# LabJunBMI/E3-invaraint-diffusion-model

Hardware: NVIDIA B200
Metric: denoiser graph-steps/s (forward + reverse-diffusion step per pocket graph; cfg2: 64 pockets x 500 steps, L=128) (higher is better)
Workload: dtype bf16

## Files before the change

### e3-invaraint-diffusion-model_b200/csrc/gemm.cu

```cuda
#include <cstdio>
#include <cstdlib>
#include <mutex>
#include <type_traits>
#include <unordered_map>

#include "common.cuh"
#include "kernels.h"

namespace seqdiff {

typedef CUresult (*PFN_encodeTiled)(CUtensorMap*, CUtensorMapDataType, cuuint32_t, void*, const cuuint64_t*,
                                    const cuuint64_t*, const cuuint32_t*, const cuuint32_t*, CUtensorMapInterleave,
                                    CUtensorMapSwizzle, CUtensorMapL2promotion, CUtensorMapFloatOOBfill);

static PFN_encodeTiled get_encode_fn() {
  static PFN_encodeTiled fn = nullptr;
  static std::once_flag once;
  std::call_once(once, [] {
    void* p = nullptr;
    cudaDriverEntryPointQueryResult qres;
    if (cudaGetDriverEntryPoint("cuTensorMapEncodeTiled", &p, cudaEnableDefault, &qres) == cudaSuccess &&
        qres == cudaDriverEntryPointSuccess)
      fn = reinterpret_cast<PFN_encodeTiled>(p);
  });
// ... 55 lines not shown
  static std::mutex mu;
  static std::unordered_map<TmapKey, CUtensorMap, TmapKeyHash> cache;
  TmapKey key{ptr, rows, cols, -32, fmt};
  {
    std::lock_guard<std::mutex> g(mu);
    auto it = cache.find(key);
    if (it != cache.end()) {
      *out = it->second;
      return SEQDIFF_OK;
    }
  }
  PFN_encodeTiled enc = get_encode_fn();
  if (!enc) {
    set_error("cuTensorMapEncodeTiled not available from the driver");
    return SEQDIFF_ERR_CUDA;
  }
  SD_CHECK((reinterpret_cast<uintptr_t>(ptr) & 15) == 0 && (cols % 32) == 0, "TMA store operand must be 16B aligned with N a multiple of 32");
  cuuint64_t gdim[2] = {static_cast<cuuint64_t>(cols), static_cast<cuuint64_t>(rows)};
  cuuint64_t gstride[1] = {static_cast<cuuint64_t>(cols) * 2};
  cuuint32_t box[2] = {32u, 32u};
  cuuint32_t estr[2] = {1u, 1u};
  CUresult r = enc(out, fmt == 1 ? CU_TENSOR_MAP_DATA_TYPE_BFLOAT16 : CU_TENSOR_MAP_DATA_TYPE_FLOAT16, 2, const_cast<void*>(ptr), gdim,
                   gstride, box, estr, CU_TENSOR_MAP_INTERLEAVE_NONE, CU_TENSOR_MAP_SWIZZLE_64B, CU_TENSOR_MAP_L2_PROMOTION_NONE,
                   CU_TENSOR_MAP_FLOAT_OOB_FILL_NONE);
  if (r != CUDA_SUCCESS) {
    set_error("cuTensorMapEncodeTiled (store) failed with CUresult " + std::to_string(static_cast<int>(r)));
    return SEQDIFF_ERR_CUDA;
  }
  std::lock_guard<std::mutex> g(mu);
  cache.emplace(key, *out);
  return SEQDIFF_OK;
}

int make_tmap_3d(const void* ptr, int fmt, int batch, int rows, int cols, int box_rows, CUtensorMap* out) {
  PFN_encodeTiled enc = get_encode_fn();
  if (!enc) {
    set_error("cuTensorMapEncodeTiled not available from the driver");
    return SEQDIFF_ERR_CUDA;
  }
  SD_CHECK((reinterpret_cast<uintptr_t>(ptr) & 15) == 0 && (cols % 8) == 0, "TMA operand must be 16B aligned with a 16B-multiple row pitch");
  cuuint64_t gdim[3] = {static_cast<cuuint64_t>(cols), static_cast<cuuint64_t>(rows), static_cast<cuuint64_t>(batch)};
  cuuint64_t gstride[2] = {static_cast<cuuint64_t>(cols) * 2, static_cast<cuuint64_t>(rows) * cols * 2};
  cuuint32_t box[3] = {64u, static_cast<cuuint32_t>(box_rows), 1u};
  cuuint32_t estr[3] = {1u, 1u, 1u};
  CUresult r = enc(out, fmt == 1 ? CU_TENSOR_MAP_DATA_TYPE_BFLOAT16 : CU_TENSOR_MAP_DATA_TYPE_FLOAT16, 3, const_cast<void*>(ptr), gdim,
                   gstride, box, estr, CU_TENSOR_MAP_INTERLEAVE_NONE, CU_TENSOR_MAP_SWIZZLE_128B, CU_TENSOR_MAP_L2_PROMOTION_L2_256B,
                   CU_TENSOR_MAP_FLOAT_OOB_FILL_NONE);
  if (r != CUDA_SUCCESS) {
    set_error("cuTensorMapEncodeTiled (3d) failed with CUresult " + std::to_string(static_cast<int>(r)));
    return SEQDIFF_ERR_CUDA;
  }
  return SEQDIFF_OK;
}

constexpr int kBM = 128;
constexpr int kBK = 64;
constexpr int kUmmaK = 16;
constexpr int kGemmThreads = 320;

template <int BN, bool CG2, bool LN = false> struct GemmCfg {
  static constexpr int kNSub = BN > 256 ? 2 : 1;
  static constexpr int kSubN = BN / kNSub;
  static constexpr int kBoxRows = CG2 ? kSubN / 2 : kSubN;
  static constexpr int kBRows = kBoxRows * kNSub;
  static constexpr int kAccStages = BN > 256 ? 1 : 2;
  static constexpr int kABytes = kBM * kBK * 2;
  static constexpr int kBBytes = kBRows * kBK * 2;
  static constexpr int kStageBytes = kABytes + kBBytes;
  static constexpr int kStages = BN > 256 ? 4 : (CG2 ? 6 : (BN == 256 ? (LN ? 3 : 4) : (BN == 192 ? 4 : (LN ? 5 : 6))));
  static constexpr int kTmemCols = BN == 128 ? 256 : 512;
  static constexpr int kStagingBytes = 8 * 32 * 32 * 4;
  static constexpr int kLnBytes = 2 * 128 * 8 + 2 * 4 * 128 * 8 + 64;
  static constexpr int kSmemBytes = kStages * kStageBytes + 1024  + 256  + kStagingBytes + (LN ? kLnBytes : 0);
  static_assert(BN <= 256 || CG2, "tiles wider than one UMMA are built for CTA pairs only");
  static_assert(kSmemBytes <= 232448, "over the 227 KB shared-memory limit");
};

template <typename T> __device__ __forceinline__ void store4(T* p, const float4& v);
template <> __device__ __forceinline__ void store4<float>(float* p, const float4& v) { *reinterpret_cast<float4*>(p) = v; }
template <> __device__ __forceinline__ void store4<bf16>(bf16* p, const float4& v) {
  *reinterpret_cast<uint2*>(p) = make_uint2(pack_bf16x2(v.x, v.y), pack_bf16x2(v.z, v.w));
}
template <> __device__ __forceinline__ void store4<f16>(f16* p, const float4& v) {
  *reinterpret_cast<uint2*>(p) = make_uint2(pack_f16x2(v.x, v.y), pack_f16x2(v.z, v.w));
}

template <typename T> __device__ __forceinline__ void add4(T*, const float4&) {}
template <> __device__ __forceinline__ void add4<float>(float* p, const float4& v) { atomicAdd(reinterpret_cast<float4*>(p), v); }

constexpr int kLnCl = 4;
struct LnOutArgs {
  const float* g;
  const float* b;
  float eps;
  void* h;
  float2* stats;
};
template <int BN, int EPI, int RESID, typename TOut, bool CG2, typename TH = void, bool TN = false>
__global__ void __launch_bounds__(kGemmThreads, 1)
gemm_tcgen05_kernel(const __grid_constant__ CUtensorMap tmA, const __grid_constant__ CUtensorMap tmB, const __grid_constant__ CUtensorMap tmC,
                    const float* __restrict__ bias, const float* __restrict__ resid, TOut* __restrict__ C, int M, int N, int K,
                    uint32_t idesc, const float2* __restrict__ ln_stats, const float* __restrict__ ln_g, const float* __restrict__ ln_b,
                    unsigned long long* __restrict__ trace, const LnOutArgs lno, int l2_stream, int ksplit) {
  constexpr bool LNOUT = !std::is_void<TH>::value;
  using Cfg = GemmCfg<BN, CG2, LNOUT>;
  static_assert(!LNOUT || (!CG2 && RESID != 0 && EPI == 0 && std::is_same<TOut, float>::value), "fused LayerNorm: 1-CTA MMA, fp32 C with residual");
  static_assert(!TN || (!CG2 && !LNOUT && RESID == 0 && EPI == 0 && std::is_same<TOut, float>::value && BN % 64 == 0 && BN <= 256), "TN: 1-CTA MMA, fp32 C");
  constexpr int STAGES = Cfg::kStages;
  constexpr int TILE_M = CG2 ? 2 * kBM : kBM;
  extern __shared__ uint8_t smem_raw[];
  uint8_t* smem = smem_raw + ((1024u - (smem_u32(smem_raw) & 1023u)) & 1023u);
  uint8_t* sA = smem;
  uint8_t* sB = smem + STAGES * Cfg::kABytes;
  uint64_t* bars = reinterpret_cast<uint64_t*>(smem + STAGES * Cfg::kStageBytes);
  uint64_t* full_bar = bars;
  uint64_t* empty_bar = bars + STAGES;
  uint64_t* tfull_bar = bars + 2 * STAGES;
  uint64_t* tempty_bar = bars + 2 * STAGES + 2;
  uint32_t* tmem_slot = reinterpret_cast<uint32_t*>(bars + 2 * STAGES + 4);

  const int warp = warp_id_uniform();
  const int lane = threadIdx.x & 31;
  const int num_n = N / BN;
  const int num_m = (M + TILE_M - 1) / TILE_M;
  const int num_tiles = num_m * num_n * ksplit;
  const int num_kb = (K + kBK - 1) / kBK;
  auto kb_lo = [&](int ks) { return static_cast<int>(static_cast<long long>(num_kb) * ks / ksplit); };
  const uint32_t cta_rank = CG2 ? cluster_ctarank() : 0u;
  const int tile0 = CG2 ? static_cast<int>(blockIdx.x >> 1) : static_cast<int>(blockIdx.x);
  const int tile_step = CG2 ? static_cast<int>(gridDim.x >> 1) : static_cast<int>(gridDim.x);
  float2* ln_cpart = reinterpret_cast<float2*>(smem + STAGES * Cfg::kStageBytes + 256 + Cfg::kStagingBytes);
  float2* ln_xpart = ln_cpart + 2 * 128;
  uint64_t* ln_bar = reinterpret_cast<uint64_t*>(ln_xpart + 2 * 4 * 128);

  int tr_n = 0;
  const bool tr_on = trace != nullptr && blockIdx.x == 0 && lane == 0 && (warp == 0 || warp == 1 || warp == 2 || warp == 6);
  const int tr_base = (warp == 0 ? 0 : warp == 1 ? 1 : warp == 2 ? 2 : 3) * 1024;
  auto TR = [&](int id) {
    if (tr_on && tr_n < 1023) trace[tr_base + 1 + tr_n++] = (static_cast<unsigned long long>(clock64()) << 8) | static_cast<unsigned>(id);
  };
  TR(40);
  if (warp == 0 && lane == 0) {
    tma_prefetch_desc(&tmA);
    tma_prefetch_desc(&tmB);
    if (!std::is_same<TOut, float>::value) tma_prefetch_desc(&tmC);
    for (int i = 0; i < STAGES; ++i) {
      mbar_init(&full_bar[i], 1);
      mbar_init(&empty_bar[i], 1);
    }
    for (int i = 0; i < 2; ++i) {
      mbar_init(&tfull_bar[i], 1);
      mbar_init(&tempty_bar[i], CG2 ? 16 : 8);
      if (LNOUT) mbar_init(&ln_bar[i], kLnCl * 128);
    }
    fence_mbar_init();
  }
  if (warp == 1) {
    if (CG2) {
      tmem_alloc_cg2(tmem_slot, Cfg::kTmemCols);
      tmem_relinquish_cg2();
    } else {
      tmem_alloc(tmem_slot, Cfg::kTmemCols);
      tmem_relinquish();
    }
  }
  tc_fence_before();
  if (CG2 || LNOUT) cluster_sync_all(); else __syncthreads();
  tc_fence_after();
  const uint32_t tmem_base = *tmem_slot;
  TR(41);
  pdl_trigger();
  pdl_wait();
  TR(42);

  if (warp == 0) {
    {
      const uint64_t pol_keep = l2_stream ? l2_policy_evict_last() : 0ull;
      int stage = 0;
      uint32_t phase = 0;
      for (int tile = tile0; tile < num_tiles; tile += tile_step) {
        const int ks = tile % ksplit, mn = tile / ksplit;
        const int m_blk = mn / num_n, n_blk = mn % num_n;
        const int a_row = m_blk * TILE_M + static_cast<int>(cta_rank) * kBM;
        for (int kb = kb_lo(ks), kb_end = kb_lo(ks + 1); kb < kb_end; ++kb) {
          mbar_wait(&empty_bar[stage], phase ^ 1);
          TR(1);
          if (CG2) {
// ... 38 lines not shown
      uint32_t phase = 0;
      int as = 0;
      uint32_t aphase = 0;
      for (int tile = tile0; tile < num_tiles; tile += tile_step) {
        mbar_wait(&tempty_bar[as], aphase ^ 1);
        tc_fence_after();
        const uint32_t tmem_d = tmem_base + static_cast<uint32_t>(as * BN);
        const int kb_begin = kb_lo(tile % ksplit), kb_end = kb_lo(tile % ksplit + 1);
        for (int kb = kb_begin; kb < kb_end; ++kb) {
          mbar_wait(&full_bar[stage], phase);
          tc_fence_after();
          TR(11);
          const uint32_t a_addr = smem_u32(sA + stage * Cfg::kABytes);
          const uint32_t b_addr = smem_u32(sB + stage * Cfg::kBBytes);
#pragma unroll
          for (int k = 0; k < kBK / kUmmaK; ++k) {
            const uint64_t adesc = TN ? umma_desc_mnmajor_sw128(a_addr + k * 2048, 8192) : umma_desc_kmajor_sw128(a_addr + k * kUmmaK * 2);
#pragma unroll
            for (int j = 0; j < Cfg::kNSub; ++j) {
              const uint64_t bdesc = TN ? umma_desc_mnmajor_sw128(b_addr + k * 2048, 8192)
                                        : umma_desc_kmajor_sw128(b_addr + j * Cfg::kBoxRows * kBK * 2 + k * kUmmaK * 2);
              if (CG2) umma_cg2_e(tmem_d + j * Cfg::kSubN, adesc, bdesc, idesc, ((kb - kb_begin) | k) != 0 ? 1u : 0u);
              else umma_bf16_e(tmem_d + j * Cfg::kSubN, adesc, bdesc, idesc, ((kb - kb_begin) | k) != 0 ? 1u : 0u);
            }
          }
          if (CG2) umma_commit_mc_e(&empty_bar[stage], 3); else umma_commit_e(&empty_bar[stage]);
          if (++stage == STAGES) { stage = 0; phase ^= 1; }
        }
        if (CG2) umma_commit_mc_e(&tfull_bar[as], 3); else umma_commit_e(&tfull_bar[as]);
        TR(12);
        if (++as == Cfg::kAccStages) { as = 0; aphase ^= 1; }
      }
    }
  } else {
    const int q = warp & 3;
    const int half = (warp - 2) >> 2;
    float* stage = reinterpret_cast<float*>(smem + STAGES * Cfg::kStageBytes + 256) + (warp - 2) * 1024;
    const int lr = lane >> 3, lc = lane & 7;
    int as = 0;
    uint32_t aphase = 0;
    int ln_it = 0;
    (void)ln_it;
    constexpr bool kTmaOut = !std::is_same<TOut, float>::value && RESID == 0;
    int pcount = 0;
    (void)pcount;
    const uint64_t pol_stream = (kTmaOut && l2_stream) ? l2_policy_evict_first() : 0ull;
    (void)pol_stream;
    constexpr int NCH = BN / 64;
    for (int tile = tile0; tile < num_tiles; tile += tile_step) {
      const int ks = tile % ksplit, mn = tile / ksplit;
      const int m_blk = mn / num_n, n_blk = mn % num_n;
      const int row_base = m_blk * TILE_M + static_cast<int>(cta_rank) * kBM + q * 32;
      SD_DEV_ASSERT(m_blk < num_m && n_blk * BN + half * (BN / 2) + (BN / 2) <= N && ks < ksplit);
      const uint32_t t_row = tmem_base + (static_cast<uint32_t>(q * 32) << 16) + static_cast<uint32_t>(as * BN) + half * (BN / 2);
      const int col0 = n_blk * BN + half * (BN / 2) + 4 * lc;
      const bool full = row_base + 32 <= M;
      float rs[LNOUT ? 8 : 1], rq[LNOUT ? 8 : 1];
      if (LNOUT) {
#pragma unroll
        for (int i = 0; i < 8; ++i) { rs[i] = 0.f; rq[i] = 0.f; }
      }
      (void)rs; (void)rq;
      if constexpr (kTmaOut) {
        const int colw = n_blk * BN + half * (BN / 2);
        uint8_t* panels = reinterpret_cast<uint8_t*>(stage);
        TR(20);
        mbar_wait(&tfull_bar[as], aphase);
        tc_fence_after();
        TR(21);
        uint32_t r[2][32];
        tmem_ld_32x32(t_row, r[0]);
#pragma unroll
        for (int ci = 0; ci < NCH; ++ci) {
          const int cur = ci & 1;
          float4 bv[8];
#pragma unroll
          for (int j4 = 0; j4 < 8; ++j4) bv[j4] = __ldg(reinterpret_cast<const float4*>(bias + colw + 32 * ci + 4 * j4));
          tmem_ld_wait();
          if (ci + 1 < NCH) tmem_ld_32x32(t_row + static_cast<uint32_t>(32 * (ci + 1)), r[cur ^ 1]);
          uint32_t pk[16];
#pragma unroll
          for (int j4 = 0; j4 < 8; ++j4) {
            float a0 = __uint_as_float(r[cur][4 * j4]) + bv[j4].x, a1 = __uint_as_float(r[cur][4 * j4 + 1]) + bv[j4].y;
            float a2 = __uint_as_float(r[cur][4 * j4 + 2]) + bv[j4].z, a3 = __uint_as_float(r[cur][4 * j4 + 3]) + bv[j4].w;
            if (EPI == 1) { a0 = gelu_fast(a0); a1 = gelu_fast(a1); a2 = gelu_fast(a2); a3 = gelu_fast(a3); }
            if (EPI == 2) { a0 = silu_fast(a0); a1 = silu_fast(a1); a2 = silu_fast(a2); a3 = silu_fast(a3); }
            pk[2 * j4] = pack2<TOut>(a0, a1);
            pk[2 * j4 + 1] = pack2<TOut>(a2, a3);
          }
          uint8_t* panel = panels + (pcount & 1) * 2048;
          if (lane == 0) tma_store_wait_read1();
          __syncwarp();
          uint8_t* prow = panel + lane * 64;
          const uint32_t sw = (smem_u32(prow) >> 7) & 3u;
#pragma unroll
// ... 54 lines not shown
#pragma unroll
        for (int jj = 0; jj < 8; ++jj)
          *reinterpret_cast<uint4*>(stage + lane * 32 + ((jj ^ (lane & 7)) << 2)) =
              make_uint4(r[tc][4 * jj], r[tc][4 * jj + 1], r[tc][4 * jj + 2], r[tc][4 * jj + 3]);
        __syncwarp();
        const int col = col0 + 32 * ci;
        auto emit_rows = [&](auto guard_tag) {
          constexpr bool kGuard = decltype(guard_tag)::value;
#pragma unroll
          for (int hh = 0; hh < 2; ++hh) {
            float4 v[4];
#pragma unroll
            for (int u = 0; u < 4; ++u) {
              const int rr = 4 * (4 * hh + u) + lr;
              v[u] = *reinterpret_cast<const float4*>(stage + rr * 32 + ((lc ^ (rr & 7)) << 2));
            }
#pragma unroll
            for (int u = 0; u < 4; ++u) {
              const int i = 4 * hh + u;
              v[u].x += b4[cur].x; v[u].y += b4[cur].y; v[u].z += b4[cur].z; v[u].w += b4[cur].w;
              if (EPI == 1) { v[u].x = gelu_fast(v[u].x); v[u].y = gelu_fast(v[u].y); v[u].z = gelu_fast(v[u].z); v[u].w = gelu_fast(v[u].w); }
              if (EPI == 2) { v[u].x = silu_fast(v[u].x); v[u].y = silu_fast(v[u].y); v[u].z = silu_fast(v[u].z); v[u].w = silu_fast(v[u].w); }
              if (RESID) {
                float4 rv = rres[i];
                if (ci + 1 < NCH) fetch_resid_row(ci + 1, i);
                if (RESID == 2) {
                  rv.x = (rv.x - st8[i].x) * st8[i].y * g4[cur].x + h4[cur].x;
                  rv.y = (rv.y - st8[i].x) * st8[i].y * g4[cur].y + h4[cur].y;
                  rv.z = (rv.z - st8[i].x) * st8[i].y * g4[cur].z + h4[cur].z;
                  rv.w = (rv.w - st8[i].x) * st8[i].y * g4[cur].w + h4[cur].w;
                }
                v[u].x += rv.x; v[u].y += rv.y; v[u].z += rv.z; v[u].w += rv.w;
              }
              if (LNOUT) {
                rs[i] += (v[u].x + v[u].y) + (v[u].z + v[u].w);
                rq[i] = fmaf(v[u].x, v[u].x, fmaf(v[u].y, v[u].y, fmaf(v[u].z, v[u].z, fmaf(v[u].w, v[u].w, rq[i]))));
              }
            }
#pragma unroll
            for (int u = 0; u < 4; ++u) {
              const int row = row_base + 4 * (4 * hh + u) + lr;
              if (!kGuard || row < M) {
                if (std::is_same<TOut, float>::value && RESID == 0 && ksplit > 1) add4(C + static_cast<size_t>(row) * N + col, v[u]);
                else store4<TOut>(C + static_cast<size_t>(row) * N + col, v[u]);
              }
            }
          }
        };
        if (full) emit_rows(std::false_type{}); else emit_rows(std::true_type{});
        __syncwarp();
      }
      }
      TR(23);
      tc_fence_before();
      __syncwarp();
      if (lane == 0) {
        if (CG2 && cta_rank != 0) mbar_arrive_cluster(mapa_u32(smem_u32(&tempty_bar[as]), 0));
        else mbar_arrive(&tempty_bar[as]);
      }
      if constexpr (LNOUT) {
        const int et = static_cast<int>(threadIdx.x) - 64;
        const int par = ln_it & 1;
        float4 vc[NCH][8];
#pragma unroll
        for (int ci = 0; ci < NCH; ++ci)
#pragma unroll
          for (int i = 0; i < 8; ++i) {
            const int row = row_base + 4 * i + lr;
            vc[ci][i] = (full || row < M) ? *reinterpret_cast<const float4*>(C + static_cast<size_t>(row) * N + col0 + 32 * ci)
                                          : make_float4(0.f, 0.f, 0.f, 0.f);
          }
#pragma unroll
        for (int i = 0; i < 8; ++i)
#pragma unroll
          for (int off = 1; off < 8; off <<= 1) {
            rs[i] += __shfl_xor_sync(0xffffffffu, rs[i], off);
            rq[i] += __shfl_xor_sync(0xffffffffu, rq[i], off);
          }
        if (lc == 0) {
#pragma unroll
          for (int i = 0; i < 8; ++i) ln_cpart[half * 128 + q * 32 + 4 * i + lr] = make_float2(rs[i], rq[i]);
        }
        asm volatile("bar.sync 1, 256;" ::: "memory");
        if (et < 128) {
          const float2 a = ln_cpart[et], b2 = ln_cpart[128 + et];
          const uint32_t my = cluster_ctarank();
#pragma unroll
          for (uint32_t pr = 0; pr < kLnCl; ++pr) {
            st_cluster_f32x2(mapa_u32(smem_u32(&ln_xpart[(par * kLnCl + static_cast<int>(my)) * 128 + et]), pr), a.x + b2.x, a.y + b2.y);
            mbar_arrive_cluster(mapa_u32(smem_u32(&ln_bar[par]), pr));
          }
        }
        TR(24);
        mbar_wait_cluster(&ln_bar[par], static_cast<uint32_t>(ln_it >> 1) & 1u);
        TR(25);
        float mean8[8], rstd8[8];
        const float inv_n = 1.0f / static_cast<float>(N);
#pragma unroll
        for (int i = 0; i < 8; ++i) {
          const int rl = q * 32 + 4 * i + lr;
          float sx = 0.f, sq = 0.f;
#pragma unroll
          for (int pr = 0; pr < kLnCl; ++pr) {
            const float2 t2 = ln_xpart[(par * kLnCl + pr) * 128 + rl];
            sx += t2.x;
            sq += t2.y;
          }
          mean8[i] = sx * inv_n;
          const float var = fmaxf(fmaf(-mean8[i], mean8[i], sq * inv_n), 0.f);
          rstd8[i] = 1.0f / sqrtf(var + lno.eps);
          if (n_blk == 0 && half == 0 && lc == 0 && row_base + 4 * i + lr < M) lno.stats[row_base + 4 * i + lr] = make_float2(mean8[i], rstd8[i]);
        }
        TH* hout = static_cast<TH*>(lno.h);
#pragma unroll
        for (int ci = 0; ci < NCH; ++ci) {
          const int col = col0 + 32 * ci;
          const float4 gg = __ldg(reinterpret_cast<const float4*>(lno.g + col));
          const float4 bb = __ldg(reinterpret_cast<const float4*>(lno.b + col));
#pragma unroll
          for (int i = 0; i < 8; ++i) {
            const int row = row_base + 4 * i + lr;
            const float4 vv = vc[ci][i];
            float4 hv;
            hv.x = (vv.x - mean8[i]) * rstd8[i] * gg.x + bb.x;
            hv.y = (vv.y - mean8[i]) * rstd8[i] * gg.y + bb.y;
            hv.z = (vv.z - mean8[i]) * rstd8[i] * gg.z + bb.z;
            hv.w = (vv.w - mean8[i]) * rstd8[i] * gg.w + bb.w;
            if (full || row < M) store4<TH>(hout + static_cast<size_t>(row) * N + col, hv);
          }
        }
        TR(26);
        ++ln_it;
      }
      if (++as == Cfg::kAccStages) { as = 0; aphase ^= 1; }
    }
    if (kTmaOut && lane == 0) tma_store_wait_all();
  }

  TR(43);
  if (tr_on) trace[tr_base] = static_cast<unsigned long long>(tr_n);
  tc_fence_before();
  if (CG2 || LNOUT) cluster_sync_all(); else __syncthreads();
  if (warp == 1) {
    tc_fence_after();
    if (CG2) tmem_dealloc_cg2(tmem_base, Cfg::kTmemCols); else tmem_dealloc(tmem_base, Cfg::kTmemCols);
  }
}

template <int BN, int EPI, int RESID, typename TOut, bool CG2>
static int launch_tc(const CUtensorMap& ta, const CUtensorMap& tb, const CUtensorMap& tc, const float* bias, const float* resid, void* C, int M,
                     int N, int K, uint32_t idesc, cudaStream_t s, const LnResid* ln = nullptr, int ksplit = 1) {
  using Cfg = GemmCfg<BN, CG2>;
  auto kfn = gemm_tcgen05_kernel<BN, EPI, RESID, TOut, CG2>;
  static bool configured = false;
  if (!configured) {
    SD_CUDA(cudaFuncSetAttribute(kfn, cudaFuncAttributeMaxDynamicSharedMemorySize, Cfg::kSmemBytes));
    configured = true;
  }
  const int tiles = ceil_div(M, CG2 ? 2 * kBM : kBM) * (N / BN) * ksplit;
  const int slots = CG2 ? num_sms() / 2 : num_sms();
  const int grid = (tiles < slots ? tiles : slots) * (CG2 ? 2 : 1);
  static const int hint_on = [] { const char* e = getenv("SEQDIFF_GEMM_L2HINT"); return e ? atoi(e) : 0; }();
  const int l2_stream = (hint_on && !std::is_same<TOut, float>::value && RESID == 0 && static_cast<double>(M) * N * 2 > 64e6) ? 1 : 0;
  SD_CUDA(launch_kc(CG2 ? 2 : 1, kfn, dim3(grid), dim3(kGemmThreads), Cfg::kSmemBytes, s, ta, tb, tc, bias, resid, static_cast<TOut*>(C), M, N, K,
                    idesc, ln ? ln->stats : nullptr, ln ? ln->g : nullptr, ln ? ln->b : nullptr, g_attn_trace, LnOutArgs{}, l2_stream, ksplit));
  SD_LAUNCHED(ksplit > 1 ? (CG2 ? "gemm_tcgen05_2cta_splitk" : "gemm_tcgen05_splitk") : (CG2 ? "gemm_tcgen05_2cta" : "gemm_tcgen05"), s);
  return SEQDIFF_OK;
}

template <int BN, int RESID, typename TH>
static int launch_tc_ln(const CUtensorMap& ta, const CUtensorMap& tb, const float* bias, const float* resid, float* C, int M, int N, int K,
                        uint32_t idesc, cudaStream_t s, const LnResid* ln, const LnOut& lo) {
  using Cfg = GemmCfg<BN, false, true>;
  auto kfn = gemm_tcgen05_kernel<BN, 0, RESID, float, false, TH>;
  static bool configured = false;
  if (!configured) {
    SD_CUDA(cudaFuncSetAttribute(kfn, cudaFuncAttributeMaxDynamicSharedMemorySize, Cfg::kSmemBytes));
    configured = true;
  }
  const int num_m = ceil_div(M, kBM);
  static int max_cl = 0;
  if (!max_cl) {
    cudaLaunchConfig_t qc{};
    qc.gridDim = dim3(num_sms() / kLnCl * kLnCl);
    qc.blockDim = dim3(kGemmThreads);
    qc.dynamicSmemBytes = Cfg::kSmemBytes;
    cudaLaunchAttribute qa[1];
    qa[0].id = cudaLaunchAttributeClusterDimension;
    qa[0].val.clusterDim.x = kLnCl;
    qa[0].val.clusterDim.y = 1;
    qa[0].val.clusterDim.z = 1;
    qc.attrs = qa;
    qc.numAttrs = 1;
    int n = 0;
    SD_CUDA(cudaOccupancyMaxActiveClusters(&n, kfn, &qc));
    max_cl = n > 0 ? n : 1;
  }
  const int waves = ceil_div(num_m, max_cl);
  const int clusters = ceil_div(num_m, waves);
  const LnOutArgs a{lo.g, lo.b, lo.eps, lo.h, lo.stats};
  SD_CUDA(launch_kc(kLnCl, kfn, dim3(clusters * kLnCl), dim3(kGemmThreads), Cfg::kSmemBytes, s, ta, tb, ta , bias, resid, C, M, N, K, idesc,
                    ln ? ln->stats : nullptr, ln ? ln->g : nullptr, ln ? ln->b : nullptr, g_attn_trace, a, 0, 1));
  SD_LAUNCHED("gemm_tcgen05_ln", s);
  return SEQDIFF_OK;
}
template <int BN, typename TH>
static int dispatch_tc_ln(const CUtensorMap& ta, const CUtensorMap& tb, const float* bias, const float* resid, float* C, int M, int N, int K,
                          uint32_t idesc, cudaStream_t s, const LnResid* ln, const LnOut& lo) {
  if (ln) return launch_tc_ln<BN, 2, TH>(ta, tb, bias, resid, C, M, N, K, idesc, s, ln, lo);
  return launch_tc_ln<BN, 1, TH>(ta, tb, bias, resid, C, M, N, K, idesc, s, ln, lo);
}

template <int BN>
static int launch_tn(const CUtensorMap& ta, const CUtensorMap& tb, const float* bias, float* C, int M, int N, int K, uint32_t idesc, int ksplit, cudaStream_t s) {
  using Cfg = GemmCfg<BN, false>;
  auto kfn = gemm_tcgen05_kernel<BN, 0, 0, float, false, void, true>;
  static bool configured = false;
  if (!configured) {
    SD_CUDA(cudaFuncSetAttribute(kfn, cudaFuncAttributeMaxDynamicSharedMemorySize, Cfg::kSmemBytes));
    configured = true;
  }
  const int tiles = ceil_div(M, kBM) * (N / BN) * ksplit;
  const int grid = tiles < num_sms() ? tiles : num_sms();
  SD_CUDA(launch_kc(1, kfn, dim3(grid), dim3(kGemmThreads), Cfg::kSmemBytes, s, ta, tb, ta, bias, static_cast<const float*>(nullptr), C, M, N, K, idesc,
                    static_cast<const float2*>(nullptr), static_cast<const float*>(nullptr), static_cast<const float*>(nullptr), g_attn_trace, LnOutArgs{}, 0, ksplit));
  SD_LAUNCHED(ksplit > 1 ? "gemm_tcgen05_tn_splitk" : "gemm_tcgen05_tn", s);
  return SEQDIFF_OK;
}
int gemm_16_tn(int M, int N, int K, const void* At, const void* Bt, int fmt, const float* bias, float* C, cudaStream_t s, int split_k) {
  SD_CHECK(M > 0 && N > 0 && K > 0, "empty GEMM");
  SD_CHECK(M % 8 == 0 && N % 128 == 0, "TN GEMM: M % 8 == 0 (16B TMA pitch) and N % 128 == 0");
  SD_CHECK((fmt | 1) == 1 && bias != nullptr, "bad operand format / bias required");
  SD_CHECK(split_k >= -1 && split_k != 0, "split_k must be -1 (auto), 1 (off) or the number of k-ranges");
  const int bn = N % 256 == 0 ? 256 : 128;
  int ksplit = split_k;
  const int nkb = ceil_div(K, kBK);
  if (ksplit < 0) {
    const int tiles = ceil_div(M, kBM) * (N / bn);
    ksplit = num_sms() / tiles;
    if (ksplit > nkb / 4) ksplit = nkb / 4;
  }
  if (ksplit > nkb) ksplit = nkb;
  if (ksplit < 1) ksplit = 1;
// ... 32 lines not shown
    if (epi == 0) return launch_tc<BN, 0, 0, bf16, CG2>(ta, tb, tc, bias, resid, C, M, N, K, idesc, s);
    if (epi == 1) return launch_tc<BN, 1, 0, bf16, CG2>(ta, tb, tc, bias, resid, C, M, N, K, idesc, s);
    return launch_tc<BN, 2, 0, bf16, CG2>(ta, tb, tc, bias, resid, C, M, N, K, idesc, s);
  }
  if (epi == 0) return launch_tc<BN, 0, 0, f16, CG2>(ta, tb, tc, bias, resid, C, M, N, K, idesc, s);
  if (epi == 1) return launch_tc<BN, 1, 0, f16, CG2>(ta, tb, tc, bias, resid, C, M, N, K, idesc, s);
  return launch_tc<BN, 2, 0, f16, CG2>(ta, tb, tc, bias, resid, C, M, N, K, idesc, s);
}

int gemm_16(int M, int N, int K, const void* A, int a_fmt, const void* W, int w_fmt, const float* bias, const float* resid, int epi,
            void* C, int out_kind, cudaStream_t s, int force_cfg, const LnResid* ln_resid, const LnOut* ln_out, int split_k) {
  SD_CHECK(M > 0 && N > 0 && K > 0, "empty GEMM");
  SD_CHECK(split_k >= -1 && split_k != 0, "split_k must be -1 (auto), 1 (off) or the number of k-ranges");
  SD_CHECK(split_k == 1 || (out_kind == 2 && !resid && !ln_out && epi == 0), "split-K accumulates into an fp32 C without residual");
  SD_CHECK(N % 128 == 0, "tcgen05 GEMM needs N % 128 == 0");
  SD_CHECK(K % 8 == 0, "tcgen05 GEMM needs K % 8 == 0 (16B TMA pitch)");
  SD_CHECK(epi >= 0 && epi <= 2, "unknown GEMM epilogue");
  SD_CHECK(!((resid || out_kind == 2) && epi != 0), "fp32 output / residual add only with the identity epilogue");
  SD_CHECK(!(resid && out_kind != 2), "a residual GEMM writes fp32");
  SD_CHECK(!ln_resid || (resid && ln_resid->stats && ln_resid->g && ln_resid->b), "LayerNorm-residual needs resid, stats and the affine");
  SD_CHECK(bias != nullptr, "bias required");
  SD_CHECK((a_fmt | 1) == 1 && out_kind >= 0 && out_kind <= 2, "bad operand format");
  SD_CHECK(a_fmt == w_fmt, "A and W must share one 16-bit format");
  if (ln_out) {
    SD_CHECK(resid && out_kind == 2 && epi == 0, "fused LayerNorm needs the fp32 residual form");
    SD_CHECK(N == 512 || N == 768 || N == 1024, "fused LayerNorm: N must be 512, 768 or 1024 (4 column quarters of 128/192/256)");
    SD_CHECK(ln_out->g && ln_out->b && ln_out->h && ln_out->stats, "fused LayerNorm: null argument");
    const int bq = N / kLnCl;
    CUtensorMap ta, tb;
    SD_TRY(make_tmap(A, a_fmt, M, K, kBM, &ta));
    SD_TRY(make_tmap(W, w_fmt, N, K, bq, &tb));
    const uint32_t idesc = umma_idesc_16(kBM, bq, static_cast<uint32_t>(a_fmt), static_cast<uint32_t>(w_fmt));
    float* Cf = static_cast<float*>(C);
#define SD_LN_DISPATCH(BN_)                                                                                                   \
  return a_fmt == 1 ? dispatch_tc_ln<BN_, bf16>(ta, tb, bias, resid, Cf, M, N, K, idesc, s, ln_resid, *ln_out)                \
                    : dispatch_tc_ln<BN_, f16>(ta, tb, bias, resid, Cf, M, N, K, idesc, s, ln_resid, *ln_out)
    if (bq == 128) { SD_LN_DISPATCH(128); }
    if (bq == 192) { SD_LN_DISPATCH(192); }
    SD_LN_DISPATCH(256);
#undef SD_LN_DISPATCH
  }
  int cfg = force_cfg;
  int ksplit = split_k;
  if (ksplit != 1 && !cfg) cfg = pick_cfg(M, N, K);
  if (!cfg) {
    static const int tune = [] { const char* e = getenv("SEQDIFF_GEMM_TUNE"); return e ? atoi(e) : 1; }();
    static std::mutex mu;
    static std::unordered_map<uint64_t, int> tuned;
    const int rkind = resid ? (ln_resid ? 2 : 1) : 0;
    const uint64_t key = (static_cast<uint64_t>(M) << 40) ^ (static_cast<uint64_t>(N) << 24) ^ (static_cast<uint64_t>(K) << 8) ^
                         (static_cast<uint64_t>(epi) << 6) ^ (static_cast<uint64_t>(out_kind) << 4) ^ (static_cast<uint64_t>(rkind) << 2) ^
                         static_cast<uint64_t>(a_fmt);
    {
      std::lock_guard<std::mutex> g(mu);
      auto it = tuned.find(key);
      if (it != tuned.end()) cfg = it->second;
    }
    if (!cfg) {
      cudaStreamCaptureStatus cap = cudaStreamCaptureStatusNone;
      SD_CUDA(cudaStreamIsCapturing(s, &cap));
      const bool can_tune = tune && cap == cudaStreamCaptureStatusNone && M > 64 && C != A && C != static_cast<const void*>(resid);
      if (!can_tune) {
        cfg = pick_cfg(M, N, K);
      } else {
        static cudaStream_t tune_streams[64] = {};
        int dev_id = 0;
        SD_CUDA(cudaGetDevice(&dev_id));
        SD_CHECK(dev_id >= 0 && dev_id < 64, "device ordinal out of range");
        if (!tune_streams[dev_id]) SD_CUDA(cudaStreamCreateWithFlags(&tune_streams[dev_id], cudaStreamNonBlocking));
// ... 171 lines not shown
```

Baseline: 33450.

## Rework fused LayerNorm GEMM epilogue with TMA residual loads and stores

Gives the fused residual+LayerNorm GEMM its own epilogue path. The fp32 residual is streamed into swizzled shared memory with TMA and double-buffered mbarriers, the summed output is written back to TMEM and stored with TMA, and the normalized bf16/f16 output goes out through TMA panels. The old path re-read C from global memory and used a single-pass sum and sum-of-squares variance. The new one computes a two-pass (Chan-style) variance from TMEM, which avoids the reload and improves numerical stability. In exchange it cuts pipeline stages for the LN configurations to make room for the staging buffers, and adds more barriers and more complex synchronisation.

After: 33430 (median of 6 runs). No clear change (-0.1%).

```diff
diff --git a/e3-invaraint-diffusion-model_b200/csrc/gemm.cu b/e3-invaraint-diffusion-model_b200/csrc/gemm.cu
--- a/e3-invaraint-diffusion-model_b200/csrc/gemm.cu
+++ b/e3-invaraint-diffusion-model_b200/csrc/gemm.cu
@@ -111,6 +111,39 @@
   return SEQDIFF_OK;
 }
 
+static int make_tmap_f32(const float* ptr, int rows, int cols, CUtensorMap* out) {
+  static std::mutex mu;
+  static std::unordered_map<TmapKey, CUtensorMap, TmapKeyHash> cache;
+  TmapKey key{ptr, rows, cols, -32, 2};
+  {
+    std::lock_guard<std::mutex> g(mu);
+    auto it = cache.find(key);
+    if (it != cache.end()) {
+      *out = it->second;
+      return SEQDIFF_OK;
+    }
+  }
+  PFN_encodeTiled enc = get_encode_fn();
+  if (!enc) {
+    set_error("cuTensorMapEncodeTiled not available from the driver");
+    return SEQDIFF_ERR_CUDA;
+  }
+  SD_CHECK((reinterpret_cast<uintptr_t>(ptr) & 15) == 0 && (cols % 32) == 0, "fp32 TMA tensor must be 16B aligned with N a multiple of 32");
+  cuuint64_t gdim[2] = {static_cast<cuuint64_t>(cols), static_cast<cuuint64_t>(rows)};
+  cuuint64_t gstride[1] = {static_cast<cuuint64_t>(cols) * 4};
+  cuuint32_t box[2] = {32u, 32u};
+  cuuint32_t estr[2] = {1u, 1u};
+  CUresult r = enc(out, CU_TENSOR_MAP_DATA_TYPE_FLOAT32, 2, const_cast<float*>(ptr), gdim, gstride, box, estr, CU_TENSOR_MAP_INTERLEAVE_NONE,
+                   CU_TENSOR_MAP_SWIZZLE_128B, CU_TENSOR_MAP_L2_PROMOTION_L2_256B, CU_TENSOR_MAP_FLOAT_OOB_FILL_NONE);
+  if (r != CUDA_SUCCESS) {
+    set_error("cuTensorMapEncodeTiled (fp32) failed with CUresult " + std::to_string(static_cast<int>(r)));
+    return SEQDIFF_ERR_CUDA;
+  }
+  std::lock_guard<std::mutex> g(mu);
+  cache.emplace(key, *out);
+  return SEQDIFF_OK;
+}
+
 int make_tmap_3d(const void* ptr, int fmt, int batch, int rows, int cols, int box_rows, CUtensorMap* out) {
   PFN_encodeTiled enc = get_encode_fn();
   if (!enc) {
@@ -146,11 +179,15 @@
   static constexpr int kABytes = kBM * kBK * 2;
   static constexpr int kBBytes = kBRows * kBK * 2;
   static constexpr int kStageBytes = kABytes + kBBytes;
-  static constexpr int kStages = BN > 256 ? 4 : (CG2 ? 6 : (BN == 256 ? (LN ? 3 : 4) : (BN == 192 ? 4 : (LN ? 5 : 6))));
+  static constexpr int kLnBoxes = 2;
+  static constexpr int kStages = LN ? (BN == 128 ? 4 : (BN == 192 ? 3 : 2))
+                                    : (BN > 256 ? 4 : (CG2 ? 6 : (BN == 256 ? 4 : (BN == 192 ? 4 : 6))));
   static constexpr int kTmemCols = BN == 128 ? 256 : 512;
-  static constexpr int kStagingBytes = 8 * 32 * 32 * 4;
-  static constexpr int kLnBytes = 2 * 128 * 8 + 2 * 4 * 128 * 8 + 64;
-  static constexpr int kSmemBytes = kStages * kStageBytes + 1024  + 256  + kStagingBytes + (LN ? kLnBytes : 0);
+  static constexpr int kBarBytes = LN ? 1024 : 256;
+  static constexpr int kLnWarpBytes = kLnBoxes * 4096 + 2048;
+  static constexpr int kStagingBytes = LN ? 8 * kLnWarpBytes : 8 * 32 * 32 * 4;
+  static constexpr int kLnBytes = 2 * 2 * 128 * 4 + 2 * 4 * 128 * 8 + (2 + 8 * kLnBoxes) * 8;
+  static constexpr int kSmemBytes = kStages * kStageBytes + 1024  + kBarBytes + kStagingBytes + (LN ? kLnBytes : 0);
   static_assert(BN <= 256 || CG2, "tiles wider than one UMMA are built for CTA pairs only");
   static_assert(kSmemBytes <= 232448, "over the 227 KB shared-memory limit");
 };
@@ -169,10 +206,12 @@
 
 constexpr int kLnCl = 4;
 struct LnOutArgs {
+  CUtensorMap tmR;
+  CUtensorMap tmO;
+  CUtensorMap tmH;
   const float* g;
   const float* b;
   float eps;
-  void* h;
   float2* stats;
 };
 template <int BN, int EPI, int RESID, typename TOut, bool CG2, typename TH = void, bool TN = false>
@@ -180,7 +219,7 @@
 gemm_tcgen05_kernel(const __grid_constant__ CUtensorMap tmA, const __grid_constant__ CUtensorMap tmB, const __grid_constant__ CUtensorMap tmC,
                     const float* __restrict__ bias, const float* __restrict__ resid, TOut* __restrict__ C, int M, int N, int K,
                     uint32_t idesc, const float2* __restrict__ ln_stats, const float* __restrict__ ln_g, const float* __restrict__ ln_b,
-                    unsigned long long* __restrict__ trace, const LnOutArgs lno, int l2_stream, int ksplit) {
+                    unsigned long long* __restrict__ trace, const __grid_constant__ LnOutArgs lno, int l2_stream, int ksplit) {
   constexpr bool LNOUT = !std::is_void<TH>::value;
   using Cfg = GemmCfg<BN, CG2, LNOUT>;
   static_assert(!LNOUT || (!CG2 && RESID != 0 && EPI == 0 && std::is_same<TOut, float>::value), "fused LayerNorm: 1-CTA MMA, fp32 C with residual");
@@ -208,8 +247,9 @@
   const uint32_t cta_rank = CG2 ? cluster_ctarank() : 0u;
   const int tile0 = CG2 ? static_cast<int>(blockIdx.x >> 1) : static_cast<int>(blockIdx.x);
   const int tile_step = CG2 ? static_cast<int>(gridDim.x >> 1) : static_cast<int>(gridDim.x);
-  float2* ln_cpart = reinterpret_cast<float2*>(smem + STAGES * Cfg::kStageBytes + 256 + Cfg::kStagingBytes);
-  float2* ln_xpart = ln_cpart + 2 * 128;
+  uint8_t* epi_smem = smem + STAGES * Cfg::kStageBytes + Cfg::kBarBytes;
+  float* ln_cpart = reinterpret_cast<float*>(epi_smem + Cfg::kStagingBytes);
+  float2* ln_xpart = reinterpret_cast<float2*>(ln_cpart + 4 * 128);
   uint64_t* ln_bar = reinterpret_cast<uint64_t*>(ln_xpart + 2 * 4 * 128);
 
   int tr_n = 0;
@@ -223,6 +263,11 @@
     tma_prefetch_desc(&tmA);
     tma_prefetch_desc(&tmB);
     if (!std::is_same<TOut, float>::value) tma_prefetch_desc(&tmC);
+    if (LNOUT) {
+      tma_prefetch_desc(&lno.tmR);
+      tma_prefetch_desc(&lno.tmO);
+      tma_prefetch_desc(&lno.tmH);
+    }
     for (int i = 0; i < STAGES; ++i) {
       mbar_init(&full_bar[i], 1);
       mbar_init(&empty_bar[i], 1);
@@ -232,6 +277,8 @@
       mbar_init(&tempty_bar[i], CG2 ? 16 : 8);
       if (LNOUT) mbar_init(&ln_bar[i], kLnCl * 128);
     }
+    if (LNOUT)
+      for (int i = 0; i < 8 * Cfg::kLnBoxes; ++i) mbar_init(&ln_bar[2 + i], 1);
     fence_mbar_init();
   }
   if (warp == 1) {
@@ -336,15 +383,197 @@
         if (++as == Cfg::kAccStages) { as = 0; aphase ^= 1; }
       }
     }
+  } else if constexpr (LNOUT) {
+    const int q = warp & 3;
+    const int ew = warp - 2;
+    const int half = ew >> 2;
+    constexpr int NCH = BN / 64;
+    constexpr int HC = BN / 2;
+    constexpr int NB = Cfg::kLnBoxes;
+    static_assert(NB >= 2 && NB <= NCH, "residual boxes per warp");
+    uint8_t* rbuf = epi_smem + ew * Cfg::kLnWarpBytes;
+    uint8_t* hpanel = rbuf + NB * 4096;
+    uint64_t* rbar = ln_bar + 2 + NB * ew;
+    float* cs = ln_cpart;
+    float* cm = ln_cpart + 256;
+    const int rl = q * 32 + lane;
+    const int colw = static_cast<int>(blockIdx.x % kLnCl) * BN + half * HC;
+    int issued = 0;
+    auto issue_upto = [&](int lim) {
+      for (; issued < lim; ++issued) {
+        const int t = tile0 + (issued / NCH) * tile_step;
+        if (t >= num_tiles) break;
+        const int b = issued % NB;
+        mbar_expect_tx_e(&rbar[b], 4096);
+        tma_load_2d_e(rbuf + b * 4096, &lno.tmR, &rbar[b], colw + 32 * (issued % NCH), (t / num_n) * kBM + q * 32);
+      }
+    };
+    issue_upto(NB);
+    int g = 0;
+    int as = 0;
+    uint32_t aphase = 0;
+    int ln_it = 0;
+    for (int tile = tile0; tile < num_tiles; tile += tile_step) {
+      const int m_blk = tile / num_n, n_blk = tile % num_n;
+      const int row_base = m_blk * kBM + q * 32;
+      const int row = row_base + lane;
+      SD_DEV_ASSERT(m_blk < num_m && n_blk * BN + half * HC == colw && colw + HC <= N && num_n == kLnCl);
+      const uint32_t t_row = tmem_base + (static_cast<uint32_t>(q * 32) << 16) + static_cast<uint32_t>(as * BN + half * HC);
+      float2 st = make_float2(0.f, 0.f);
+      if (RESID == 2 && row < M) st = __ldg(ln_stats + row);
+      TR(20);
+      mbar_wait(&tfull_bar[as], aphase);
+      tc_fence_after();
+      TR(21);
+      uint32_t r[32];
+      float rsum = 0.f;
+#pragma unroll 1
+      for (int ci = 0; ci < NCH; ++ci, ++g) {
+        const int b = g % NB;
+        const int col = colw + 32 * ci;
+        tmem_ld_32x32(t_row + static_cast<uint32_t>(32 * ci), r);
+        mbar_wait(&rbar[b], static_cast<uint32_t>(g / NB) & 1u);
+        tmem_ld_wait();
+        uint8_t* box_row = rbuf + b * 4096 + lane * 128;
+#pragma unroll
+        for (int j = 0; j < 8; ++j) {
+          float4* p4 = reinterpret_cast<float4*>(box_row + ((j ^ (lane & 7)) << 4));
+          float4 rv = *p4;
+          const float4 bv = __ldg(reinterpret_cast<const float4*>(bias + col + 4 * j));
+          if (RESID == 2) {
+            const float4 gv = __ldg(reinterpret_cast<const float4*>(ln_g + col + 4 * j));
+            const float4 hv = __ldg(reinterpret_cast<const float4*>(ln_b + col + 4 * j));
+            rv.x = (rv.x - st.x) * st.y * gv.x + hv.x;
+            rv.y = (rv.y - st.x) * st.y * gv.y + hv.y;
+            rv.z = (rv.z - st.x) * st.y * gv.z + hv.z;
+            rv.w = (rv.w - st.x) * st.y * gv.w + hv.w;
+          }
+          float4 v;
+          v.x = (__uint_as_float(r[4 * j]) + bv.x) + rv.x;
+          v.y = (__uint_as_float(r[4 * j + 1]) + bv.y) + rv.y;
+          v.z = (__uint_as_float(r[4 * j + 2]) + bv.z) + rv.z;
+          v.w = (__uint_as_float(r[4 * j + 3]) + bv.w) + rv.w;
+          rsum += v.x;
+          rsum += v.y;
+          rsum += v.z;
+          rsum += v.w;
+          r[4 * j] = __float_as_uint(v.x);
+          r[4 * j + 1] = __float_as_uint(v.y);
+          r[4 * j + 2] = __float_as_uint(v.z);
+          r[4 * j + 3] = __float_as_uint(v.w);
+          *p4 = v;
+        }
+        tmem_st_32x32(t_row + static_cast<uint32_t>(32 * ci), r);
+        fence_proxy_async_smem();
+        __syncwarp();
+        if (lane == 0) {
+          tma_store_2d(&lno.tmO, rbuf + b * 4096, col, row_base);
+          tma_store_commit();
+          tma_store_wait_read1();
+        }
+        __syncwarp();
+        issue_upto(g + NB);
+      }
+      tmem_st_wait();
+      TR(23);
+      cs[half * 128 + rl] = rsum;
+      asm volatile("bar.sync 1, 256;" ::: "memory");
+      const float s_cta = cs[rl] + cs[128 + rl];
+      const float mean_cta = s_cta / static_cast<float>(BN);
+      float m2 = 0.f;
+#pragma unroll
+      for (int ci = 0; ci < NCH; ++ci) {
+        tmem_ld_32x32(t_row + static_cast<uint32_t>(32 * ci), r);
+        tmem_ld_wait();
+#pragma unroll
+        for (int j = 0; j < 32; ++j) {
+          const float d = __uint_as_float(r[j]) - mean_cta;
+          m2 = fmaf(d, d, m2);
+        }
+      }
+      cm[half * 128 + rl] = m2;
+      if (lane == 0) tma_store_wait_read();
+      __syncwarp();
+      issue_upto(g + NB);
+      asm volatile("bar.sync 1, 256;" ::: "memory");
+      const int par = ln_it & 1;
+      if (half == 0) {
+        const float m2_cta = cm[rl] + cm[128 + rl];
+        const uint32_t my = cluster_ctarank();
+#pragma unroll
+        for (uint32_t pr = 0; pr < kLnCl; ++pr) {
+          st_cluster_f32x2(mapa_u32(smem_u32(&ln_xpart[(par * kLnCl + static_cast<int>(my)) * 128 + rl]), pr), s_cta, m2_cta);
+          mbar_arrive_cluster(mapa_u32(smem_u32(&ln_bar[par]), pr));
+        }
+      }
+      TR(24);
+      mbar_wait_cluster(&ln_bar[par], static_cast<uint32_t>(ln_it >> 1) & 1u);
+      TR(25);
+      float2 part[kLnCl];
+      float sum = 0.f;
+#pragma unroll
+      for (int pr = 0; pr < kLnCl; ++pr) {
+        part[pr] = ln_xpart[(par * kLnCl + pr) * 128 + rl];
+        sum += part[pr].x;
+      }
+      const float mean = sum / static_cast<float>(N);
+      float m2_all = 0.f;
+#pragma unroll
+      for (int pr = 0; pr < kLnCl; ++pr) {
+        const float d = part[pr].x / static_cast<float>(BN) - mean;
+        m2_all += part[pr].y + static_cast<float>(BN) * d * d;
+      }
+      const float rstd = 1.0f / sqrtf(m2_all / static_cast<float>(N) + lno.eps);
+      if (n_blk == 0 && half == 0 && row < M) lno.stats[row] = make_float2(mean, rstd);
+#pragma unroll 1
+      for (int ci = 0; ci < NCH; ++ci) {
+        const int col = colw + 32 * ci;
+        tmem_ld_32x32(t_row + static_cast<uint32_t>(32 * ci), r);
+        tmem_ld_wait();
+        if (ci + 1 == NCH) {
+          tc_fence_before();
+          __syncwarp();
+          if (lane == 0) mbar_arrive(&tempty_bar[as]);
+        }
+        uint32_t pk[16];
+#pragma unroll
+        for (int j = 0; j < 8; ++j) {
+          const float4 gv = __ldg(reinterpret_cast<const float4*>(lno.g + col + 4 * j));
+          const float4 bv = __ldg(reinterpret_cast<const float4*>(lno.b + col + 4 * j));
+          const float h0 = (__uint_as_float(r[4 * j]) - mean) * rstd * gv.x + bv.x;
+          const float h1 = (__uint_as_float(r[4 * j + 1]) - mean) * rstd * gv.y + bv.y;
+          const float h2 = (__uint_as_float(r[4 * j + 2]) - mean) * rstd * gv.z + bv.z;
+          const float h3 = (__uint_as_float(r[4 * j + 3]) - mean) * rstd * gv.w + bv.w;
+          pk[2 * j] = pack2<TH>(h0, h1);
+          pk[2 * j + 1] = pack2<TH>(h2, h3);
+        }
+        if (lane == 0) tma_store_wait_read();
+        __syncwarp();
+        uint8_t* prow = hpanel + lane * 64;
+        const uint32_t sw = (smem_u32(prow) >> 7) & 3u;
+#pragma unroll
+        for (int c16 = 0; c16 < 4; ++c16)
+          *reinterpret_cast<uint4*>(prow + ((static_cast<uint32_t>(c16) ^ sw) << 4)) =
+              make_uint4(pk[4 * c16], pk[4 * c16 + 1], pk[4 * c16 + 2], pk[4 * c16 + 3]);
+        fence_proxy_async_smem();
+        __syncwarp();
+        if (lane == 0) {
+          tma_store_2d(&lno.tmH, hpanel, col, row_base);
+          tma_store_commit();
+        }
+      }
+      TR(26);
+      ++ln_it;
+      if (++as == Cfg::kAccStages) { as = 0; aphase ^= 1; }
+    }
+    if (lane == 0) tma_store_wait_all();
   } else {
     const int q = warp & 3;
     const int half = (warp - 2) >> 2;
-    float* stage = reinterpret_cast<float*>(smem + STAGES * Cfg::kStageBytes + 256) + (warp - 2) * 1024;
+    float* stage = reinterpret_cast<float*>(epi_smem) + (warp - 2) * 1024;
     const int lr = lane >> 3, lc = lane & 7;
     int as = 0;
     uint32_t aphase = 0;
-    int ln_it = 0;
-    (void)ln_it;
     constexpr bool kTmaOut = !std::is_same<TOut, float>::value && RESID == 0;
     int pcount = 0;
     (void)pcount;
@@ -359,12 +588,6 @@
       const uint32_t t_row = tmem_base + (static_cast<uint32_t>(q * 32) << 16) + static_cast<uint32_t>(as * BN) + half * (BN / 2);
       const int col0 = n_blk * BN + half * (BN / 2) + 4 * lc;
       const bool full = row_base + 32 <= M;
-      float rs[LNOUT ? 8 : 1], rq[LNOUT ? 8 : 1];
-      if (LNOUT) {
-#pragma unroll
-        for (int i = 0; i < 8; ++i) { rs[i] = 0.f; rq[i] = 0.f; }
-      }
-      (void)rs; (void)rq;
       if constexpr (kTmaOut) {
         const int colw = n_blk * BN + half * (BN / 2);
         uint8_t* panels = reinterpret_cast<uint8_t*>(stage);
@@ -485,10 +708,6 @@
                 }
                 v[u].x += rv.x; v[u].y += rv.y; v[u].z += rv.z; v[u].w += rv.w;
               }
-              if (LNOUT) {
-                rs[i] += (v[u].x + v[u].y) + (v[u].z + v[u].w);
-                rq[i] = fmaf(v[u].x, v[u].x, fmaf(v[u].y, v[u].y, fmaf(v[u].z, v[u].z, fmaf(v[u].w, v[u].w, rq[i]))));
-              }
             }
 #pragma unroll
             for (int u = 0; u < 4; ++u) {
@@ -511,80 +730,6 @@
         if (CG2 && cta_rank != 0) mbar_arrive_cluster(mapa_u32(smem_u32(&tempty_bar[as]), 0));
         else mbar_arrive(&tempty_bar[as]);
       }
-      if constexpr (LNOUT) {
-        const int et = static_cast<int>(threadIdx.x) - 64;
-        const int par = ln_it & 1;
-        float4 vc[NCH][8];
-#pragma unroll
-        for (int ci = 0; ci < NCH; ++ci)
-#pragma unroll
-          for (int i = 0; i < 8; ++i) {
-            const int row = row_base + 4 * i + lr;
-            vc[ci][i] = (full || row < M) ? *reinterpret_cast<const float4*>(C + static_cast<size_t>(row) * N + col0 + 32 * ci)
-                                          : make_float4(0.f, 0.f, 0.f, 0.f);
-          }
-#pragma unroll
-        for (int i = 0; i < 8; ++i)
-#pragma unroll
-          for (int off = 1; off < 8; off <<= 1) {
-            rs[i] += __shfl_xor_sync(0xffffffffu, rs[i], off);
-            rq[i] += __shfl_xor_sync(0xffffffffu, rq[i], off);
-          }
-        if (lc == 0) {
-#pragma unroll
-          for (int i = 0; i < 8; ++i) ln_cpart[half * 128 + q * 32 + 4 * i + lr] = make_float2(rs[i], rq[i]);
-        }
-        asm volatile("bar.sync 1, 256;" ::: "memory");
-        if (et < 128) {
-          const float2 a = ln_cpart[et], b2 = ln_cpart[128 + et];
-          const uint32_t my = cluster_ctarank();
-#pragma unroll
-          for (uint32_t pr = 0; pr < kLnCl; ++pr) {
-            st_cluster_f32x2(mapa_u32(smem_u32(&ln_xpart[(par * kLnCl + static_cast<int>(my)) * 128 + et]), pr), a.x + b2.x, a.y + b2.y);
-            mbar_arrive_cluster(mapa_u32(smem_u32(&ln_bar[par]), pr));
-          }
-        }
-        TR(24);
-        mbar_wait_cluster(&ln_bar[par], static_cast<uint32_t>(ln_it >> 1) & 1u);
-        TR(25);
-        float mean8[8], rstd8[8];
-        const float inv_n = 1.0f / static_cast<float>(N);
-#pragma unroll
-        for (int i = 0; i < 8; ++i) {
-          const int rl = q * 32 + 4 * i + lr;
-          float sx = 0.f, sq = 0.f;
-#pragma unroll
-          for (int pr = 0; pr < kLnCl; ++pr) {
-            const float2 t2 = ln_xpart[(par * kLnCl + pr) * 128 + rl];
-            sx += t2.x;
-            sq += t2.y;
-          }
-          mean8[i] = sx * inv_n;
-          const float var = fmaxf(fmaf(-mean8[i], mean8[i], sq * inv_n), 0.f);
-          rstd8[i] = 1.0f / sqrtf(var + lno.eps);
-          if (n_blk == 0 && half == 0 && lc == 0 && row_base + 4 * i + lr < M) lno.stats[row_base + 4 * i + lr] = make_float2(mean8[i], rstd8[i]);
-        }
-        TH* hout = static_cast<TH*>(lno.h);
-#pragma unroll
-        for (int ci = 0; ci < NCH; ++ci) {
-          const int col = col0 + 32 * ci;
-          const float4 gg = __ldg(reinterpret_cast<const float4*>(lno.g + col));
-          const float4 bb = __ldg(reinterpret_cast<const float4*>(lno.b + col));
-#pragma unroll
-          for (int i = 0; i < 8; ++i) {
-            const int row = row_base + 4 * i + lr;
-            const float4 vv = vc[ci][i];
-            float4 hv;
-            hv.x = (vv.x - mean8[i]) * rstd8[i] * gg.x + bb.x;
-            hv.y = (vv.y - mean8[i]) * rstd8[i] * gg.y + bb.y;
-            hv.z = (vv.z - mean8[i]) * rstd8[i] * gg.z + bb.z;
-            hv.w = (vv.w - mean8[i]) * rstd8[i] * gg.w + bb.w;
-            if (full || row < M) store4<TH>(hout + static_cast<size_t>(row) * N + col, hv);
-          }
-        }
-        TR(26);
-        ++ln_it;
-      }
       if (++as == Cfg::kAccStages) { as = 0; aphase ^= 1; }
     }
     if (kTmaOut && lane == 0) tma_store_wait_all();
@@ -623,7 +768,7 @@
 
 template <int BN, int RESID, typename TH>
 static int launch_tc_ln(const CUtensorMap& ta, const CUtensorMap& tb, const float* bias, const float* resid, float* C, int M, int N, int K,
-                        uint32_t idesc, cudaStream_t s, const LnResid* ln, const LnOut& lo) {
+                        uint32_t idesc, cudaStream_t s, const LnResid* ln, const LnOutArgs& a) {
   using Cfg = GemmCfg<BN, false, true>;
   auto kfn = gemm_tcgen05_kernel<BN, 0, RESID, float, false, TH>;
   static bool configured = false;
@@ -651,7 +796,6 @@
   }
   const int waves = ceil_div(num_m, max_cl);
   const int clusters = ceil_div(num_m, waves);
-  const LnOutArgs a{lo.g, lo.b, lo.eps, lo.h, lo.stats};
   SD_CUDA(launch_kc(kLnCl, kfn, dim3(clusters * kLnCl), dim3(kGemmThreads), Cfg::kSmemBytes, s, ta, tb, ta , bias, resid, C, M, N, K, idesc,
                     ln ? ln->stats : nullptr, ln ? ln->g : nullptr, ln ? ln->b : nullptr, g_attn_trace, a, 0, 1));
   SD_LAUNCHED("gemm_tcgen05_ln", s);
@@ -659,9 +803,9 @@
 }
 template <int BN, typename TH>
 static int dispatch_tc_ln(const CUtensorMap& ta, const CUtensorMap& tb, const float* bias, const float* resid, float* C, int M, int N, int K,
-                          uint32_t idesc, cudaStream_t s, const LnResid* ln, const LnOut& lo) {
-  if (ln) return launch_tc_ln<BN, 2, TH>(ta, tb, bias, resid, C, M, N, K, idesc, s, ln, lo);
-  return launch_tc_ln<BN, 1, TH>(ta, tb, bias, resid, C, M, N, K, idesc, s, ln, lo);
+                          uint32_t idesc, cudaStream_t s, const LnResid* ln, const LnOutArgs& a) {
+  if (ln) return launch_tc_ln<BN, 2, TH>(ta, tb, bias, resid, C, M, N, K, idesc, s, ln, a);
+  return launch_tc_ln<BN, 1, TH>(ta, tb, bias, resid, C, M, N, K, idesc, s, ln, a);
 }
 
 template <int BN>
@@ -760,9 +904,17 @@
     SD_TRY(make_tmap(W, w_fmt, N, K, bq, &tb));
     const uint32_t idesc = umma_idesc_16(kBM, bq, static_cast<uint32_t>(a_fmt), static_cast<uint32_t>(w_fmt));
     float* Cf = static_cast<float*>(C);
+    LnOutArgs la{};
+    SD_TRY(make_tmap_f32(resid, M, N, &la.tmR));
+    SD_TRY(make_tmap_f32(Cf, M, N, &la.tmO));
+    SD_TRY(make_tmap_store16(ln_out->h, a_fmt, M, N, &la.tmH));
+    la.g = ln_out->g;
+    la.b = ln_out->b;
+    la.eps = ln_out->eps;
+    la.stats = ln_out->stats;
 #define SD_LN_DISPATCH(BN_)                                                                                                   \
-  return a_fmt == 1 ? dispatch_tc_ln<BN_, bf16>(ta, tb, bias, resid, Cf, M, N, K, idesc, s, ln_resid, *ln_out)                \
-                    : dispatch_tc_ln<BN_, f16>(ta, tb, bias, resid, Cf, M, N, K, idesc, s, ln_resid, *ln_out)
+  return a_fmt == 1 ? dispatch_tc_ln<BN_, bf16>(ta, tb, bias, resid, Cf, M, N, K, idesc, s, ln_resid, la)                     \
+                    : dispatch_tc_ln<BN_, f16>(ta, tb, bias, resid, Cf, M, N, K, idesc, s, ln_resid, la)
     if (bq == 128) { SD_LN_DISPATCH(128); }
     if (bq == 192) { SD_LN_DISPATCH(192); }
     SD_LN_DISPATCH(256);
```
